# lRomul/ball-action-spotting

Hardware: AMD Instinct MI355X
Metric: frame-windows/sec (fwd+bwd) at 15x736x1280, batch 4 (higher is better)
Workload: dtype bf16; 1 GPU; sampling_weights_001: 4x15x736x1280 windows/GPU, fwd + focal loss + bwd + grad all-reduce + AdamW (mds.train fused focal loss / multi-tensor optimizer); global_batch=4, parallelism=dp1

## Files before the change

### ball-action-spotting_amd/csrc/k_pw.hip

```cpp
#include <stdlib.h>
#include "gemm.h"

#define PW_BM 128
#ifndef MDS_PW_GPRE3
#define MDS_PW_GPRE3 1
#endif
#define PW_BN 128
#define PW_SP 72

template <typename T> struct PwCfg;
template <> struct PwCfg<bf16_t> { static const int KC = 64, LD = 80; };
template <> struct PwCfg<float> { static const int KC = 32, LD = 40; };

template <typename T, int PRO, int WN, int BM, int TAIL, bool SPLIT = false, bool DEEP = false>
__global__ __launch_bounds__(256, (WN == 2 && BM == 128) || TAIL == 1 || SPLIT || DEEP ? 2 : 3) void pw_fwd_kernel(mds_pw_fwd_args a) {
  MDS_CHAIN_PRIO();
  static_assert(!DEEP || (TAIL != 1 && (PRO == MDS_PRO_NONE || PRO == MDS_PRO_GATE) && WN == 2 && BM == 64), "DEEP variants");
  static_assert(!SPLIT || (TAIL != 1 && (PRO == MDS_PRO_NONE || PRO == MDS_PRO_GATE) && WN == 2 && BM == 64), "SPLIT variants");
  constexpr bool POST = TAIL == 1, EPI = TAIL == 2;
  typedef typename Frag<T>::type frag_t;
  typedef Mma<T, EPI && sizeof(T) == 4 && MDS_EVAL_X3> MM;
  constexpr int KC = PwCfg<T>::KC, LD = PwCfg<T>::LD, VPR = KC / 8, RPP = 256 / VPR, NL = BM / RPP;
  constexpr int BN = 64 * WN, MFW = (WN == 2 ? BM / 32 : BM / 64), NLW = BN / RPP;
  MDS_DYN_SMEM(smem);
// ... 203 lines not shown
        const int last = t == (int)gridDim.z - 1;
        if (last) atomicExch(tk, 0);
        *lastp = last;
      }
      __syncthreads();
      const bool last = *lastp != 0;
      __syncthreads();
      if (!last) continue;
#pragma unroll
      for (int mf = 0; mf < MFW; ++mf)
#pragma unroll
        for (int nf = 0; nf < 4; ++nf) acc[mf][nf] = (f32x4){0.f, 0.f, 0.f, 0.f};
      for (int z0 = 0; z0 < (int)gridDim.z; z0 += 4) {
        f32x4 t[4][MFW][4];
#pragma unroll
        for (int zz = 0; zz < 4; ++zz)
#pragma unroll
          for (int mf = 0; mf < MFW; ++mf) {
            const long m = m0 + 16 * MFW * wm + 16 * mf + i;
            const bool ok = m < a.M && z0 + zz < (int)gridDim.z;
            const float* prow = a.split_part + (long)(z0 + zz) * MN + m * N + n0 + 64 * wn + 4 * q;
#pragma unroll
            for (int nf = 0; nf < 4; ++nf) t[zz][mf][nf] = (ok && nf < nfr) ? ld_coherent4(prow + 16 * nf) : (f32x4){0.f, 0.f, 0.f, 0.f};
          }
#pragma unroll
        for (int zz = 0; zz < 4; ++zz)
#pragma unroll
          for (int mf = 0; mf < MFW; ++mf)
#pragma unroll
            for (int nf = 0; nf < 4; ++nf) acc[mf][nf] += t[zz][mf][nf];
      }
    }

    float ps[16], pss[16];
#pragma unroll
    for (int e = 0; e < 16; ++e) { ps[e] = 0.f; pss[e] = 0.f; }
    float* pbn = (float*)smem;
    if (POST) {
      __syncthreads();
      if (tid < BN) {
#pragma unroll
        for (int k = 0; k < 4; ++k) pbn[k * BN + tid] = pb[k];
      }
      __syncthreads();
    }
    if (EPI) {
      __syncthreads();
      if (tid < BN) { pbn[tid] = pb[0]; pbn[BN + tid] = pb[1]; }
      __syncthreads();
    }
#pragma unroll
    for (int mf = 0; mf < MFW; ++mf) {
      const long m = m0 + 16 * MFW * wm + 16 * mf + i;
      const bool ok = m < a.M;
      T* yrow = y + (ok ? m : 0) * N + n0 + 64 * wn + 4 * q;
      float v[4][4];
#pragma unroll
      for (int nf = 0; nf < 4; ++nf)
#pragma unroll
        for (int r = 0; r < 4; ++r) v[nf][r] = acc[mf][nf][r];
      if (EPI) {
#pragma unroll
        for (int nf = 0; nf < 4; ++nf) {
          const float* pc = pbn + 64 * wn + 16 * nf + 4 * q;
          const f32x4 sc = *(const f32x4*)pc, sh = *(const f32x4*)(pc + BN);
#pragma unroll
          for (int r = 0; r < 4; ++r) {
            const float z = v[nf][r] * sc[r] + sh[r];
            v[nf][r] = a.epi.mode == MDS_EPI_BN_SILU ? siluf_(z) : z;
          }
        }
      }
      if (a.residual && ok) {
        const T* rrow = (const T*)a.residual + m * N + n0 + 64 * wn + 4 * q;
#pragma unroll
        for (int nf = 0; nf < 4; ++nf) {
          if (nf < nfr) {
            float rr[4];
            load4(rrow + 16 * nf, rr);
#pragma unroll
            for (int r = 0; r < 4; ++r) v[nf][r] += rr[r];
          }
        }
      }
      if (POST) {
        const float mk = (a.post.mode == MDS_POST_MASK) ? a.post.mask[(unsigned)(ok ? m : 0) / (unsigned)a.post.rows_per_group] : 1.0f;
#pragma unroll
        for (int nf = 0; nf < 4; ++nf) {
          if (nf < nfr) {
            const float ys[4] = {rys[mf][nf].get(0), rys[mf][nf].get(1), rys[mf][nf].get(2), rys[mf][nf].get(3)};
            const float* pc = pbn + 64 * wn + 16 * nf + 4 * q;
            const f32x4 mu = *(const f32x4*)(pc + 2 * BN), rs = *(const f32x4*)(pc + 3 * BN);
            if (a.post.mode == MDS_POST_SILU) {
              const f32x4 sc = *(const f32x4*)pc, sh = *(const f32x4*)(pc + BN);
#pragma unroll
              for (int r = 0; r < 4; ++r) v[nf][r] *= silu_gradf_(ys[r] * sc[r] + sh[r]);
            }
#pragma unroll
            for (int r = 0; r < 4; ++r) {
              const float g = Elem<T>::rnd(v[nf][r]) * mk;
              ps[nf * 4 + r] += g;
              pss[nf * 4 + r] += g * ((ys[r] - mu[r]) * rs[r]);
            }
          }
        }
      }
      if (STG) {
#pragma unroll
        for (int nf = 0; nf < 4; ++nf) store4(stg + i * PW_SP + 16 * nf + 4 * q, v[nf]);
        wave_lds_sync();
        T* ybase = y + (m0 + 16 * MFW * wm + 16 * mf) * N + n0 + 64 * wn;
#pragma unroll
        for (int t = 0; t < 2; ++t) {
          const int vv = lane + 64 * t, row = vv >> 3, c = vv & 7;
          if (m0 + 16 * MFW * wm + 16 * mf + row < a.M && (c >> 1) < nfr) {
            RawV8<T> o;
            o.ld(stg + row * PW_SP + 8 * c);
            o.st(ybase + (long)row * N + 8 * c);
          }
        }
        wave_lds_sync();
      } else if (ok) {
#pragma unroll
        for (int nf = 0; nf < 4; ++nf)
          if (nf < nfr) store4(yrow + 16 * nf, v[nf]);
      }
      if (!POST) {
#pragma unroll
        for (int nf = 0; nf < 4; ++nf)
#pragma unroll
          for (int r = 0; r < 4; ++r) { ps[nf * 4 + r] += v[nf][r]; pss[nf * 4 + r] += v[nf][r] * v[nf][r]; }
      }
    }
    if (POST ? (a.post.stats != nullptr) : (a.stats != nullptr)) {
      const int e = reduce_scatter16(ps, i);
      reduce_scatter16(pss, i);
      const int n = n0 + 64 * wn + 16 * (e >> 2) + 4 * q + (e & 3);
      if (n < N) {
        const long so = (long)((blockIdx.x + wm) % MDS_STAT_SLOTS) * 2 * N;
        if (POST) {
          atomicAdd(a.post.stats + so + n, (double)ps[0]);
          atomicAdd(a.post.stats + so + N + n, (double)pss[0]);
        } else {
          atomicAdd(a.stats + so + n, (double)ps[0]);
          atomicAdd(a.stats + so + N + n, (double)pss[0]);
        }
      }
    }
  }
}

int pw_fwd_wres_try(const mds_pw_fwd_args* a, mds_stream_t stream);
int pw_fwd_k_try(const mds_pw_fwd_args* a, mds_stream_t stream);

int c3_pw_try(const mds_pw_fwd_args* a, mds_stream_t stream);

extern "C" int mds_pw_fwd(const mds_pw_fwd_args* a, mds_stream_t stream) {
  MDS_REQUIRE(a && a->M > 0 && a->K > 0 && a->N > 0, "pw_fwd: bad dims");
  MDS_REQUIRE(a->K % 8 == 0 && a->N % 16 == 0, "pw_fwd: K=%d must be a multiple of 8, N=%d of 16", a->K, a->N);
  MDS_REQUIRE(a->x && a->w && a->y, "pw_fwd: null pointer");
  MDS_REQUIRE(a->pro.mode == MDS_PRO_NONE || a->pro.mode == MDS_PRO_GATE || (a->pro.scale && a->pro.shift), "pw_fwd: prologue needs scale/shift");
  MDS_REQUIRE((a->pro.mode != MDS_PRO_BN_SILU_GATE && a->pro.mode != MDS_PRO_GATE) || (a->pro.gate && a->pro.rows_per_group > 0), "pw_fwd: gate prologue");
  const bool post = a->post.mode != MDS_POST_NONE;
  const bool epi = a->epi.mode != MDS_EPI_NONE;
  if (epi) {
    MDS_REQUIRE(a->epi.scale && a->epi.shift && !a->stats && !post, "pw_fwd: an output transform needs scale/shift and excludes statistics and post statistics");
    MDS_REQUIRE(a->pro.mode == MDS_PRO_NONE || a->pro.mode == MDS_PRO_GATE || a->pro.mode == MDS_PRO_BN_SILU, "pw_fwd: an output transform takes the NONE, GATE or BN_SILU prologue");
  }
  if (post) {
    MDS_REQUIRE(a->post.y && a->post.bn && a->post.stats && !a->stats, "pw_fwd: post statistics need y, bn, stats (and no forward stats)");
    MDS_REQUIRE(a->post.mode != MDS_POST_MASK || (a->post.mask && a->post.rows_per_group > 0), "pw_fwd: post mask");
    MDS_REQUIRE(a->pro.mode == MDS_PRO_NONE && a->M < 4294967295L, "pw_fwd: post statistics are a data-gradient feature (no forward prologue)");
  }
  const bool split = a->split > 1;
  if (split) {
    MDS_REQUIRE(a->split <= MDS_PW_MAX_SPLIT && a->split_part && a->split_ticket, "pw_fwd: split-K needs split <= %d, a partial buffer and tickets", MDS_PW_MAX_SPLIT);
    MDS_REQUIRE(!post && !a->stats && (a->pro.mode == MDS_PRO_NONE || a->pro.mode == MDS_PRO_GATE),
                "pw_fwd: split-K is an inference-plan feature (NONE / GATE prologue, no statistics, no post statistics)");
  }
  if (!split && c3_pw_try(a, stream)) return mds_check_launch("pw_fwd");
  if (!split) { const int rc = pw_fwd_k_try(a, stream); if (rc <= 0) return rc; }
  if (!split) { const int rc = pw_fwd_wres_try(a, stream); if (rc <= 0) return rc; }
  const int wn = (a->N <= 64 && !split) ? 1 : 2;
  const int BN = 64 * wn;
  const long bar64 = mds_knob(MDS_KNOB_PW_BM64) > 0 ? 1000L * mds_knob(MDS_KNOB_PW_BM64) : 400000;
  const int bm = (wn == 2 && a->M <= bar64) ? 64 : PW_BM;
  MDS_REQUIRE(!split || bm == 64, "pw_fwd: split-K is for small M (64-row tiles)");
  const int mt = cdiv(a->M, bm), nt = cdiv(a->N, BN);
  int gy = 1;
  if (nt > 1) { gy = cdiv(mds_knob(MDS_KNOB_PW_GY) > 0 ? mds_knob(MDS_KNOB_PW_GY) : 1536, mt); if (gy > nt) gy = nt; if (gy < 1) gy = 1; }
  dim3 grid(mt, gy, split ? a->split : 1), block(256);
  const int kchunks = cdiv(split ? cdiv(a->K, a->split) : a->K, PwCfg<float>::KC);
  const bool deep = a->dtype == MDS_F32 && (epi || split) && wn == 2 && bm == 64 && kchunks >= 3 &&
                    (long)mt * gy * (split ? a->split : 1) <= 256 && mds_knob(MDS_KNOB_PW_DEEP) != 1;
#define PW_GOSPLIT(T, PRO, TAIL_) \
  do { const size_t smem = (size_t)(bm + BN) * PwCfg<T>::LD * sizeof(T) + (sizeof(T) == 2 ? 4 * 16 * PW_SP * 2 : 0); \
       if (sizeof(T) == 4 && deep) MDS_LAUNCH((pw_fwd_kernel<T, PRO, 2, 64, TAIL_, true, sizeof(T) == 4>), grid, block, smem, stream, *a); \
       else MDS_LAUNCH((pw_fwd_kernel<T, PRO, 2, 64, TAIL_, true>), grid, block, smem, stream, *a); } while (0)
#define PW_GODEEP(T, PRO) \
  do { const size_t smem = (size_t)(bm + BN) * PwCfg<T>::LD * sizeof(T) + (sizeof(T) == 2 ? 4 * 16 * PW_SP * 2 : 0); \
       MDS_LAUNCH((pw_fwd_kernel<T, PRO, 2, 64, 2, false, sizeof(T) == 4>), grid, block, smem, stream, *a); } while (0)
#define PW_GO2(T, PRO, TAIL_) \
  do { const size_t smem = (size_t)(bm + BN) * PwCfg<T>::LD * sizeof(T) + (sizeof(T) == 2 ? 4 * 16 * PW_SP * 2 : 0); \
       if (wn == 2 && bm == 64) MDS_LAUNCH((pw_fwd_kernel<T, PRO, 2, 64, TAIL_>), grid, block, smem, stream, *a); \
       else if (wn == 2) MDS_LAUNCH((pw_fwd_kernel<T, PRO, 2, 128, TAIL_>), grid, block, smem, stream, *a); \
       else MDS_LAUNCH((pw_fwd_kernel<T, PRO, 1, 128, TAIL_>), grid, block, smem, stream, *a); } while (0)
#define PW_GO(T, PRO) PW_GO2(T, PRO, 0)
  MDS_DISPATCH_DTYPE(a->dtype, T, {
    if (split) {
      if (epi) { if (a->pro.mode == MDS_PRO_GATE) PW_GOSPLIT(T, MDS_PRO_GATE, 2); else PW_GOSPLIT(T, MDS_PRO_NONE, 2); }
      else { if (a->pro.mode == MDS_PRO_GATE) PW_GOSPLIT(T, MDS_PRO_GATE, 0); else PW_GOSPLIT(T, MDS_PRO_NONE, 0); }
    }
    else if (post) PW_GO2(T, MDS_PRO_NONE, 1);
    else if (epi && deep && sizeof(T) == 4 && (a->pro.mode == MDS_PRO_GATE || a->pro.mode == MDS_PRO_NONE)) {
      if (a->pro.mode == MDS_PRO_GATE) PW_GODEEP(T, MDS_PRO_GATE); else PW_GODEEP(T, MDS_PRO_NONE);
    }
    else if (epi) { if (a->pro.mode == MDS_PRO_GATE) PW_GO2(T, MDS_PRO_GATE, 2); else if (a->pro.mode == MDS_PRO_BN_SILU) PW_GO2(T, MDS_PRO_BN_SILU, 2); else PW_GO2(T, MDS_PRO_NONE, 2); }
    else switch (a->pro.mode) {
      case MDS_PRO_NONE: PW_GO(T, MDS_PRO_NONE); break;
      case MDS_PRO_AFFINE: PW_GO(T, MDS_PRO_AFFINE); break;
      case MDS_PRO_BN_SILU: PW_GO(T, MDS_PRO_BN_SILU); break;
      case MDS_PRO_BN_SILU_GATE: PW_GO(T, MDS_PRO_BN_SILU_GATE); break;
      case MDS_PRO_GATE: PW_GO(T, MDS_PRO_GATE); break;
      default: mds_set_error("pw_fwd: prologue mode %d", a->pro.mode); return MDS_ERR_BAD_ARG;
    }
  });
#undef PW_GO
#undef PW_GO2
#undef PW_GOSPLIT
#undef PW_GODEEP
  return mds_check_launch("pw_fwd");
}

extern "C" int mds_pw_fwd_split(long M, int K, int N, int dtype) {
  const int knob = mds_knob(MDS_KNOB_PW_SPLIT);
  if (knob == 1 || M <= 0 || K <= 0 || N <= 0) return 1;
  const int kc = dtype == MDS_BF16 ? PwCfg<bf16_t>::KC : PwCfg<float>::KC;
  const long chunks = cdiv(K, kc), tiles = cdiv(M, MDS_PW_SPLIT_TILE_ROWS) * cdiv(N, 128);
  if (tiles >= 100 || chunks < 16) return 1;
  long s = knob >= 2 ? knob : 4;
  if (s > chunks / 3) s = chunks / 3;
  if (s > MDS_PW_MAX_SPLIT) s = MDS_PW_MAX_SPLIT;
  return s < 2 ? 1 : (int)s;
}

#define WG_ROWS 64
template <typename T> struct WgCfg;
template <> struct WgCfg<bf16_t> { static const int MW = 2, LDT = WG_ROWS + 8; };
template <> struct WgCfg<float> { static const int MW = 1, LDT = WG_ROWS + 4; };
template <int LDT> MDS_DEV int wg_off(int c, int m) { return c * LDT + 8 * ((m >> 3) ^ ((c >> 3) & 7)) + (m & 7); }
MDS_DEV void wg_put(bf16_t* base, int off, float v0, float v1) {
  *(uint32_t*)(base + off) = pack2(v0, v1);
}
MDS_DEV void wg_put(float* base, int off, float v0, float) { base[off] = v0; }

template <typename T, int PRO, int NF, int KF>
__global__ __launch_bounds__(256, 2) void pw_wgrad_kernel(mds_pw_wgrad_args a, int rows_per_block) {
  typedef typename Frag<T>::type frag_t;
  constexpr int MW = WgCfg<T>::MW, LDT = WgCfg<T>::LDT;
  constexpr int NT = 64 * NF, KT = 16 * KF, XCH = KT / 8, YCH = NT / 8;
  constexpr int XN = (WG_ROWS / MW) * XCH, YN = (WG_ROWS / MW) * YCH;
  constexpr int XI = (XN + 255) / 256, YI = (YN + 255) / 256;
  MDS_DYN_SMEM(smem);
  T* xsT = (T*)smem;
  T* dsT = xsT + KT * LDT;
  const int tid = threadIdx.x, lane = tid & 63, wave = MDS_UNIFORM(tid >> 6);
  const int i = lane & 15, q = lane >> 4;
  const int K = a.K, N = a.N;
  const int ntiles_k = (K + KT - 1) / KT;
  const int n0 = (blockIdx.y / ntiles_k) * NT, kt0 = (blockIdx.y % ntiles_k) * KT;
  const long mbeg = (long)blockIdx.x * rows_per_block;
  long mend = mbeg + rows_per_block;
  if (mend > a.M) mend = a.M;
  const T* x = (const T*)a.x;
  const T* dy = (const T*)a.dy;
  const int kfr = (K - kt0 >= KT) ? KF : ((K - kt0 + 15) >> 4);

  constexpr bool FIXED_CH = (256 % XCH) == 0;
  float sc[8], sh[8];
  if (FIXED_CH && PRO != MDS_PRO_NONE && PRO != MDS_PRO_GATE) {
    const int kx = kt0 + 8 * (tid % XCH);
    if (kx < K) { load8f(a.pro.scale + kx, sc); load8f(a.pro.shift + kx, sh); }
  }

  f32x4 acc[NF][KF];
#pragma unroll
  for (int u = 0; u < NF; ++u)
#pragma unroll
    for (int v = 0; v < KF; ++v) acc[u][v] = (f32x4){0.f, 0.f, 0.f, 0.f};

  RawV8<T> rx[XI][MW], ry[YI][MW];
  auto issue = [&](long mb) {
#pragma unroll
    for (int p = 0; p < XI; ++p) {
      const int it = tid + 256 * p, kx = kt0 + 8 * (it % XCH);
#pragma unroll
      for (int h = 0; h < MW; ++h) {
        const long m = mb + (it / XCH) * MW + h;
        if (it < XN && m < mend && kx < K) rx[p][h].ld(x + m * K + kx); else rx[p][h].zero();
      }
    }
#pragma unroll
    for (int p = 0; p < YI; ++p) {
      const int it = tid + 256 * p, n = n0 + 8 * (it % YCH);
#pragma unroll
      for (int h = 0; h < MW; ++h) {
        const long m = mb + (it / YCH) * MW + h;
        if (it < YN && m < mend && n < N) ry[p][h].ld(dy + m * N + n); else ry[p][h].zero();
      }
    }
  };
  issue(mbeg);
  for (long mb = mbeg; mb < mend; mb += WG_ROWS) {
    __syncthreads();
#pragma unroll
    for (int p = 0; p < XI; ++p) {
      const int it = tid + 256 * p, xc = it % XCH, kx = kt0 + 8 * xc;
      if (it < XN) {
        float v[MW][8];
#pragma unroll
        for (int h = 0; h < MW; ++h) {
          const long m = mb + (it / XCH) * MW + h;
          rx[p][h].get(v[h]);
          if (PRO != MDS_PRO_NONE && m < mend && kx < K) {
            if (PRO != MDS_PRO_GATE) {
              float scl[8], shl[8];
              if (!FIXED_CH) { load8f(a.pro.scale + kx, scl); load8f(a.pro.shift + kx, shl); }
#pragma unroll
              for (int j = 0; j < 8; ++j) {
                float z = v[h][j] * (FIXED_CH ? sc[j] : scl[j]) + (FIXED_CH ? sh[j] : shl[j]);
                v[h][j] = (PRO == MDS_PRO_AFFINE) ? z : siluf_(z);
              }
            }
            if (PRO == MDS_PRO_BN_SILU_GATE || PRO == MDS_PRO_GATE) {
// ... 268 lines not shown
```

### ball-action-spotting_amd/csrc/k_pwk8.hip

```cpp
#include <stdlib.h>
#include <type_traits>
#include "gemm.h"

namespace {
template <int V> using ic = std::integral_constant<int, V>;

template <int MFW, int WM, int NFW, int WN, int DX, int PRO, int TAIL>
__global__ __launch_bounds__(512) void pwk8_kernel(mds_pw_fwd_args a) {
  MDS_CHAIN_PRIO();
  static_assert(WM * WN == 4, "four consumer waves");
  constexpr bool XF = PRO != MDS_PRO_NONE;
  constexpr int NEED = XF ? 2 : 1;
  static_assert(DX >= NEED + 2, "at least one DMA batch stays in flight over a barrier");
  constexpr bool HAS_BN = PRO == MDS_PRO_AFFINE || PRO == MDS_PRO_BN_SILU || PRO == MDS_PRO_BN_SILU_GATE;
  constexpr bool HAS_ACT = PRO == MDS_PRO_BN_SILU || PRO == MDS_PRO_BN_SILU_GATE;
  constexpr bool HAS_GATE = PRO == MDS_PRO_BN_SILU_GATE || PRO == MDS_PRO_GATE;
  constexpr int BM = 16 * MFW * WM, BNP = 16 * NFW * WN;
  constexpr int NB = BM / 8;
  constexpr int XS = BM * 128, RX = DX + 1;
  constexpr int DW = 3;
  MDS_DYN_SMEM(smem);
  const lds_t xring = lds_addr_of(smem);
  const int tid = threadIdx.x, lane = tid & 63, wave = MDS_UNIFORM(tid >> 6);
  const long m0 = (long)blockIdx.x * BM;
// ... 204 lines not shown
    for (int nf = 0; nf < NFW; ++nf) {
      int f = wn * NFW + nf;
      if (f >= NFT) f = NFT - 1;
      wfp[nf] = (const bf16_t*)a.w_frag + (long)f * 512 + lane * 8;
    }
    const long wstep = (long)NFT * 512;
    u16x8 wf[4][NFW];
    int wk = 0;
    auto load_w = [&](auto Pc) {
      constexpr int P = decltype(Pc)::value;
      const int kk = wk < KST ? wk : KST - 1;
#pragma unroll
      for (int nf = 0; nf < NFW; ++nf) gld16(wf[P][nf], wfp[nf] + kk * wstep);
      ++wk;
    };
    const lds_t fo0 = wm * MFW * 2048 + i * 128 + ((q ^ (i & 7)) << 4), fo1 = wm * MFW * 2048 + i * 128 + (((4 + q) ^ (i & 7)) << 4);
    u16x8 xf[2][MFW];
    int csx = 0;

    load_w(ic<0>()); load_w(ic<1>()); load_w(ic<2>());
    for (int t = -NEED; t < 0; ++t) raw_barrier();
#pragma unroll
    for (int mf = 0; mf < MFW; ++mf) xf[0][mf] = lds_ld16(xring + mf * 2048 + fo0);

    auto kstep = [&](auto Pc, auto KSc, lds_t nxt, int s) {
      constexpr int P = decltype(Pc)::value, KS = decltype(KSc)::value;
      PWK_STAMP(s + NEED, 3 * KS);
      wait_vm<(DW - 1) * NFW>();
      wait_lgkm0();
      PWK_STAMP(s + NEED, 3 * KS + 1);
#pragma unroll
      for (int nf = 0; nf < NFW; ++nf) reg_pin(wf[P][nf]);
#pragma unroll
      for (int mf = 0; mf < MFW; ++mf) reg_pin(xf[KS][mf]);
      MDS_SCHED_FENCE();
      load_w(ic<(P + DW) & 3>());
      MDS_SCHED_FENCE();
#pragma unroll
      for (int nf = 0; nf < NFW; ++nf)
#pragma unroll
        for (int mf = 0; mf < MFW; ++mf) {
          mma16(wf[P][nf], xf[KS][mf], acc[mf][nf]);
          if (nf == 0) xf[KS ^ 1][mf] = lds_ld16(nxt + mf * 2048 + (KS ? fo0 : fo1));
          MDS_SCHED_FENCE();
        }
      PWK_STAMP(s + NEED, 3 * KS + 2);
    };
    auto stage = [&](int s, auto SPc) {
      constexpr int SP = decltype(SPc)::value;
      const lds_t xb = xring + csx * XS;
      int nsx = csx + 1;
      if (nsx == RX) nsx = 0;
      const lds_t xn = xring + nsx * XS;
      const bool last = s == S - 1, two = !(ktail && last);
      kstep(ic<2 * SP>(), ic<0>(), xb, s);
      raw_barrier();
      if (two) kstep(ic<2 * SP + 1>(), ic<1>(), xn, s);
      csx = nsx;
    };
    for (int s = 0; s < S; s += 2) {
      stage(s, ic<0>());
      if (s + 1 < S) stage(s + 1, ic<1>());
    }
    PWK_STAMP(S + NEED, 0);
    wait_vm<0>();
    wait_lgkm0();
  }
#ifdef PWK_TRACE
  raw_barrier();
  if (trc) {
    const unsigned long long* tl = (const unsigned long long*)(smem + RX * XS);
    for (int e = tid; e < (S + NEED + 1) * 64; e += 512) ((unsigned long long*)a.split_part)[e] = tl[e];
  }
  PWK_STAMP(S + NEED + 1, 0);
#endif

  raw_barrier();
  constexpr int SP = BNP + 4;
  float* stage_f = (float*)smem;
  if (wave < 4) {
    const int i = lane & 15, q = lane >> 4;
    const int wm = wave / WN, wn = wave % WN;
#pragma unroll
    for (int mf = 0; mf < MFW; ++mf)
#pragma unroll
      for (int nf = 0; nf < NFW; ++nf)
        *(f32x4*)(stage_f + (16 * (wm * MFW + mf) + i) * SP + 16 * (wn * NFW + nf) + 4 * q) = acc[mf][nf];
  }
  __syncthreads();
  if (rg < RG) {
#pragma unroll
    for (int jj = 0; jj < JMAX; ++jj) {
      const int rr = rg + RG * jj;
      const long m = m0 + rr;
      if (rr < BM && m < a.M) {
        const f32x4 lo4 = *(const f32x4*)(stage_f + rr * SP + 8 * c), hi4 = *(const f32x4*)(stage_f + rr * SP + 8 * c + 4);
        float v[8] = {lo4[0], lo4[1], lo4[2], lo4[3], hi4[0], hi4[1], hi4[2], hi4[3]};
        if (DG) {
#pragma unroll
          for (int j = 0; j < 8; ++j) {
            v[j] += bf2f(rres[jj][j]);
            if (post) {
              const float ys = bf2f(rys[jj][j]);
              if (a.post.mode == MDS_POST_SILU) v[j] *= silu_gradf_(ys * pb[0][j] + pb[1][j]);
              const float g = Elem<bf16_t>::rnd(v[j]) * rmk[jj];
              cs[j] += g;
              css[j] += g * ((ys - pb[2][j]) * pb[3][j]);
            }
          }
        } else {
#pragma unroll
          for (int j = 0; j < 8; ++j) { cs[j] += v[j]; css[j] += v[j] * v[j]; }
        }
        *(u16x8*)(y + m * N + 8 * c) = pack8(v);
      }
    }
  }
  if (sdst) {
    float* red = stage_f + BM * SP;
    if (rg < RG) {
      float* rp = red + (long)rg * 2 * N + 8 * c;
      *(f32x4*)rp = (f32x4){cs[0], cs[1], cs[2], cs[3]};
      *(f32x4*)(rp + 4) = (f32x4){cs[4], cs[5], cs[6], cs[7]};
      *(f32x4*)(rp + N) = (f32x4){css[0], css[1], css[2], css[3]};
      *(f32x4*)(rp + N + 4) = (f32x4){css[4], css[5], css[6], css[7]};
    }
    __syncthreads();
    double* sl = sdst + (long)(blockIdx.x % MDS_STAT_SLOTS) * 2 * N;
    for (int e = tid; e < 2 * N; e += 512) {
      float t = 0.f;
      for (int g = 0; g < RG; ++g) t += red[g * 2 * N + e];
      atomicAdd(sl + e, (double)t);
    }
  }
}

template <int MFW, int WM, int NFW, int WN, int DX>
size_t pwk8_smem(int N) {
  const int BM = 16 * MFW * WM, BNP = 16 * NFW * WN;
  size_t ring = (size_t)(DX + 1) * BM * 128;
#ifdef PWK_TRACE
  ring += 16 * 1024;
#endif
  const int RG = 512 / (N >> 3);
  const size_t epi = ((size_t)BM * (BNP + 4) + (size_t)RG * 2 * N) * 4;
  return ring > epi ? ring : epi;
}

bool pwk8_shape_ok(long M, int K, int N, int dtype) {
  return dtype == MDS_BF16 && K % 32 == 0 && K >= 64 && N % 16 == 0 && N <= 192 && N > 64 && M < 4294967295L;
}
}

extern "C" int mds_pw_fwd_wants_frag(long M, int K, int N, int dtype, int data_gradient) {
  const int knob = mds_knob(MDS_KNOB_PWK);
  if (knob == 1 || !pwk8_shape_ok(M, K, N, dtype)) return 0;
  if (knob == 2) return 1;
  if ((knob == 0 && data_gradient) || (knob == 4 && !data_gradient)) return 0;
  return K >= N && K >= 128 && N > 128 && M >= 4096 && M <= 40000;
}

int pw_fwd_k_try(const mds_pw_fwd_args* a, mds_stream_t stream) {
  if (!a->w_frag || a->epi.mode != MDS_EPI_NONE || a->split > 1) return 1;
  const int N = a->N, mode = a->pro.mode;
  const bool post = a->post.mode != MDS_POST_NONE;
  const bool dg = a->form ? a->form == 2 : (post || a->residual != nullptr);
  if (!dg && (post || a->residual != nullptr)) return 1;
  if (!mds_pw_fwd_wants_frag(a->M, a->K, a->N, a->dtype, dg)) return 1;
  if (dg && (mode != MDS_PRO_NONE || a->stats)) return 1;
  const int shape = N > 128 ? 0 : (N > 96 ? 1 : 2);
  const int cus = mds_cu_count();
  auto cost = [&](int bm) { const long blocks = cdiv(a->M, bm); return (long)cdiv(blocks, cus) * bm; };
  int BM;
  if (shape == 2) BM = 96;
  else { BM = 64; for (int bm : {80, 96, 128}) if (cost(bm) < cost(BM) && !(dg && bm > (shape == 0 ? 80 : 96))) BM = bm; }
  const int kb = mds_knob(MDS_KNOB_PWK_BM);
  if (kb > 0 && shape != 2 && (kb == 64 || kb == 80 || ((kb == 96 || kb == 128) && !(dg && kb > (shape == 0 ? 80 : 96))))) BM = kb;
  const bool gated = mode == MDS_PRO_BN_SILU_GATE || mode == MDS_PRO_GATE;
  if (gated && a->pro.rows_per_group < BM) return 1;
  const dim3 grid(cdiv(a->M, BM)), block(512);
#define PWK_GO(MFW, WM, NFW, WN, DX, PRO, TAIL)                                                                  \
  do { const size_t smem = pwk8_smem<MFW, WM, NFW, WN, DX>(N);                                                   \
       MDS_LAUNCH((pwk8_kernel<MFW, WM, NFW, WN, DX, PRO, TAIL>), grid, block, smem, stream, *a); } while (0)
#define PWK_ROWS(NFW, WN, DX, PRO, TAIL)                                                                         \
  do { if (BM == 64) PWK_GO(4, 1, NFW, WN, DX, PRO, TAIL); else if (BM == 80) PWK_GO(5, 1, NFW, WN, DX, PRO, TAIL); \
       else if (BM == 96) PWK_GO(6, 1, NFW, WN, DX, PRO, TAIL); else PWK_GO(8, 1, NFW, WN, DX, PRO, TAIL); } while (0)
#define PWK_SHAPE(DX, PRO, TAIL)                                                                                 \
  do { if (shape == 0) PWK_ROWS(3, 4, DX, PRO, TAIL); else if (shape == 1) PWK_ROWS(2, 4, DX, PRO, TAIL);        \
       else PWK_GO(3, 2, 3, 2, DX, PRO, TAIL); } while (0)
  if (dg) {
    if (shape == 2) PWK_GO(3, 2, 3, 2, 6, MDS_PRO_NONE, 1);
    else if (BM == 64) { if (shape == 0) PWK_GO(4, 1, 3, 4, 6, MDS_PRO_NONE, 1); else PWK_GO(4, 1, 2, 4, 6, MDS_PRO_NONE, 1); }
    else if (BM == 80) { if (shape == 0) PWK_GO(5, 1, 3, 4, 6, MDS_PRO_NONE, 1); else PWK_GO(5, 1, 2, 4, 6, MDS_PRO_NONE, 1); }
    else PWK_GO(6, 1, 2, 4, 6, MDS_PRO_NONE, 1);
  }
  else switch (mode) {
    case MDS_PRO_NONE: PWK_SHAPE(6, MDS_PRO_NONE, 0); break;
    case MDS_PRO_AFFINE: PWK_SHAPE(7, MDS_PRO_AFFINE, 0); break;
    case MDS_PRO_BN_SILU: PWK_SHAPE(7, MDS_PRO_BN_SILU, 0); break;
    case MDS_PRO_BN_SILU_GATE: PWK_SHAPE(7, MDS_PRO_BN_SILU_GATE, 0); break;
    default: PWK_SHAPE(7, MDS_PRO_GATE, 0); break;
  }
#undef PWK_SHAPE
#undef PWK_ROWS
#undef PWK_GO
  return mds_check_launch("pw_fwd (K-streaming)");
}
```

### include/mds.h

```cpp
#ifndef MDS_H
#define MDS_H
#ifdef __cplusplus
extern "C" {
#endif

#define MDS_VERSION 133
#define MDS_F32 0
#define MDS_BF16 1
#define MDS_STAT_SLOTS 32

#define MDS_ERR_BAD_ARG (-1)
#define MDS_ERR_UNSUPPORTED (-2)
#define MDS_ERR_LAUNCH (-3)

typedef void* mds_stream_t;

int mds_version(void);
const char* mds_last_error(void);
#define MDS_KNOB_CONV_BLOCKS 0
#define MDS_KNOB_DW_ORDER 1
#define MDS_KNOB_PW_WRES 2
#define MDS_KNOB_WG_DBG 4
#define MDS_KNOB_WG_BLOCKS 5
#define MDS_KNOB_DW3_L 7
#define MDS_KNOB_STREAM_BLOCKS 8
#define MDS_KNOB_DW2_L 9
#define MDS_KNOB_PW_SPLIT 10
#define MDS_KNOB_DW2_R 11
#define MDS_KNOB_PW_GY 12
#define MDS_KNOB_PW_BM64 13
#define MDS_KNOB_REDUCE_PASSES 14
#define MDS_KNOB_DW2_BLOCKS 15
#define MDS_KNOB_REDUCE_BLOCKS 16
#define MDS_KNOB_PW_DEEP 17
#define MDS_KNOB_PWK 18
#define MDS_KNOB_PWK_BM 19
#define MDS_KNOB_STEM_FWD 20
#define MDS_KNOB_DW3G 21
#define MDS_KNOB_C3 22
#define MDS_KNOB_C3_BWD_BLOCKS 24
#define MDS_KNOB_COUNT 25
int mds_dev_set(int knob, int value);
int mds_launch_event(void* event);

#define MDS_EPI_NONE 0
#define MDS_EPI_AFFINE 1
#define MDS_EPI_BN_SILU 2
typedef struct {
  int mode;
  const float* scale;
  const float* shift;
} mds_epi_t;

#define MDS_PRO_NONE 0
#define MDS_PRO_AFFINE 1
#define MDS_PRO_BN_SILU 2
#define MDS_PRO_BN_SILU_GATE 3
#define MDS_PRO_GATE 4
typedef struct {
  int mode;
  const float* scale;
  const float* shift;
  const float* gate;
  long rows_per_group;
} mds_pro_t;

#define MDS_G_PLAIN 0
#define MDS_G_SILU 1
#define MDS_G_SE_SILU 2
#define MDS_G_MASK 3
typedef struct {
  int mode;
  const void* u;
  const float* gate;
  const float* dpooled;
  const float* mask;
  long rows_per_group;
} mds_gsrc_t;

typedef struct {
  int mode;
  mds_gsrc_t g;
  const void* y;
  const float* bn;
  const float* lin;
} mds_dyp_t;

#define MDS_POST_NONE 0
#define MDS_POST_PLAIN 1
#define MDS_POST_MASK 2
#define MDS_POST_SILU 3
typedef struct {
  int mode;
  const void* y;
  const float* bn;
  const float* mask;
  long rows_per_group;
  double* stats;
} mds_poststat_t;

typedef struct {
  int dtype;
  long M;
  int K, N;
  const void* x;
  const void* w;
  void* y;
  mds_pro_t pro;
  const void* residual;
  double* stats;
  mds_poststat_t post;
  mds_epi_t epi;
  const void* w_frag;
  int split;
  float* split_part;
  int* split_ticket;
  int form;
} mds_pw_fwd_args;
int mds_pw_fwd(const mds_pw_fwd_args* a, mds_stream_t stream);
int mds_pw_fwd_split(long M, int K, int N, int dtype);
int mds_pw_fwd_wants_frag(long M, int K, int N, int dtype, int data_gradient);
#define MDS_PW_MAX_SPLIT 16
#define MDS_PW_SPLIT_TILE_ROWS 64
#define MDS_PW_SPLIT_TICKET_STRIDE 32

typedef struct {
  int dtype;
  long M;
  int K, N;
  const void* x;
  const void* dy;
  float* dw;
  mds_pro_t pro;
} mds_pw_wgrad_args;
int mds_pw_wgrad(const mds_pw_wgrad_args* a, mds_stream_t stream);

#define MDS_MAX_TAPS 9
typedef struct {
  int dtype;
  int N, IH, IW, Cin;
  int OH, OW, Cout;
  int A, B;
  int oy0, ox0, os;
  int is;
  int ntaps;
  int dy[MDS_MAX_TAPS], dx[MDS_MAX_TAPS], wi[MDS_MAX_TAPS];
  int wtaps;
  const void* x;
  const void* w;
  void* y;
  mds_pro_t pro;
  const void* residual;
  double* stats;
  int ngroups;
  int g_ntaps[4], g_oy0[4], g_ox0[4], g_A[4], g_B[4];
  mds_epi_t epi;
  mds_poststat_t post;
} mds_conv_fwd_args;
int mds_conv_fwd(const mds_conv_fwd_args* a, mds_stream_t stream);
int mds_conv_dgrad_post_ok(int dtype, int N, int IH, int IW, int Cin, int Cout, int stride, int has_residual);

typedef struct {
  int dtype;
  int N, IH, IW, Cin, OH, OW, Cout;
  int is, ntaps;
  int dy[MDS_MAX_TAPS], dx[MDS_MAX_TAPS], wi[MDS_MAX_TAPS];
  int wtaps;
  const void* x;
  const void* dyt;
  float* dw;
  mds_pro_t pro;
} mds_conv_wgrad_args;
int mds_conv_wgrad(const mds_conv_wgrad_args* a, mds_stream_t stream);

typedef struct {
  const unsigned char* u8;
  int nsrc, src_h, src_w;
  int pad_top, pad_left;
  float scale;
} mds_ingest_t;
typedef struct {
  int dtype;
  int N, H, W, OH, OW, Cout;
  int pad_t, pad_l;
  const float* x;
  const void* w;
  void* y;
  double* stats;
  mds_ingest_t ingest;
  mds_epi_t epi;
} mds_stem_fwd_args;
int mds_stem_fwd(const mds_stem_fwd_args* a, mds_stream_t stream);

typedef struct {
// ... 396 lines not shown
```

Before: 334.4 frame-windows/s.

## Add row-stationary pointwise GEMM kernel for small-K, wide-N expansion layers

Adds a new pointwise forward kernel that keeps a tile of input rows (K of 96 to 192) resident in registers and streams weight fragments through a register ring, looping over all output column tiles. Each output tile is staged through double-buffered LDS so global stores are coalesced, and per-channel BN statistics are accumulated in LDS and flushed once per block. This targets expansion convolutions with N of 384 or more, where reloading the input for each column tile is wasteful. The frag-weight request now also covers these shapes. The cost is extra dispatch logic and a new template set with MFW/KST variants.

```diff
diff --git a/ball-action-spotting_amd/csrc/k_pw.hip b/ball-action-spotting_amd/csrc/k_pw.hip
--- a/ball-action-spotting_amd/csrc/k_pw.hip
+++ b/ball-action-spotting_amd/csrc/k_pw.hip
@@ -379,6 +379,7 @@
 
 int pw_fwd_wres_try(const mds_pw_fwd_args* a, mds_stream_t stream);
 int pw_fwd_k_try(const mds_pw_fwd_args* a, mds_stream_t stream);
+int pw_fwd_x_try(const mds_pw_fwd_args* a, mds_stream_t stream);
 
 int c3_pw_try(const mds_pw_fwd_args* a, mds_stream_t stream);
 
@@ -407,6 +408,7 @@
   }
   if (!split && c3_pw_try(a, stream)) return mds_check_launch("pw_fwd");
   if (!split) { const int rc = pw_fwd_k_try(a, stream); if (rc <= 0) return rc; }
+  if (!split) { const int rc = pw_fwd_x_try(a, stream); if (rc <= 0) return rc; }
   if (!split) { const int rc = pw_fwd_wres_try(a, stream); if (rc <= 0) return rc; }
   const int wn = (a->N <= 64 && !split) ? 1 : 2;
   const int BN = 64 * wn;
diff --git a/ball-action-spotting_amd/csrc/k_pwk8.hip b/ball-action-spotting_amd/csrc/k_pwk8.hip
--- a/ball-action-spotting_amd/csrc/k_pwk8.hip
+++ b/ball-action-spotting_amd/csrc/k_pwk8.hip
@@ -380,12 +380,18 @@
 }
 }
 
-extern "C" int mds_pw_fwd_wants_frag(long M, int K, int N, int dtype, int data_gradient) {
+int pw_fwd_x_wants(long M, int K, int N, int dtype, int data_gradient);
+
+static int pwk8_wants(long M, int K, int N, int dtype, int data_gradient) {
   const int knob = mds_knob(MDS_KNOB_PWK);
   if (knob == 1 || !pwk8_shape_ok(M, K, N, dtype)) return 0;
   if (knob == 2) return 1;
   if ((knob == 0 && data_gradient) || (knob == 4 && !data_gradient)) return 0;
   return K >= N && K >= 128 && N > 128 && M >= 4096 && M <= 40000;
+}
+
+extern "C" int mds_pw_fwd_wants_frag(long M, int K, int N, int dtype, int data_gradient) {
+  return pwk8_wants(M, K, N, dtype, data_gradient) || pw_fwd_x_wants(M, K, N, dtype, data_gradient);
 }
 
 int pw_fwd_k_try(const mds_pw_fwd_args* a, mds_stream_t stream) {
@@ -394,7 +400,7 @@
   const bool post = a->post.mode != MDS_POST_NONE;
   const bool dg = a->form ? a->form == 2 : (post || a->residual != nullptr);
   if (!dg && (post || a->residual != nullptr)) return 1;
-  if (!mds_pw_fwd_wants_frag(a->M, a->K, a->N, a->dtype, dg)) return 1;
+  if (!pwk8_wants(a->M, a->K, a->N, a->dtype, dg)) return 1;
   if (dg && (mode != MDS_PRO_NONE || a->stats)) return 1;
   const int shape = N > 128 ? 0 : (N > 96 ? 1 : 2);
   const int cus = mds_cu_count();
diff --git a/ball-action-spotting_amd/csrc/k_pwx.hip b/ball-action-spotting_amd/csrc/k_pwx.hip
--- /dev/null
+++ b/ball-action-spotting_amd/csrc/k_pwx.hip
@@ -0,0 +1,199 @@
+#include <stdlib.h>
+#include <type_traits>
+#include "gemm.h"
+
+namespace {
+template <int MFW, int KST>
+struct PwxCfg {
+  static constexpr int BM = 16 * MFW, S = (KST + 1) / 2;
+  static constexpr int R = 2 * KST, DW = R - 1;
+  static constexpr int SPT = (BM * 16 + 511) / 512;
+  static constexpr int XB = S * BM * 128;
+  static constexpr int SP = 272;
+  static constexpr int STG = BM * SP;
+};
+
+template <int MFW, int KST>
+__global__ __launch_bounds__(512) void pwx_kernel(mds_pw_fwd_args a) {
+  MDS_CHAIN_PRIO();
+  typedef PwxCfg<MFW, KST> C;
+  constexpr int BM = C::BM, S = C::S, R = C::R, DW = C::DW, SPT = C::SPT;
+  MDS_DYN_SMEM(smem);
+  const lds_t xlds = lds_addr_of(smem);
+  char* const stg = smem + C::XB;
+  float* const red = (float*)(stg + 2 * C::STG);
+  const int tid = threadIdx.x, lane = tid & 63, wave = MDS_UNIFORM(tid >> 6);
+  const int i = lane & 15, q = lane >> 4;
+  const long m0 = (long)blockIdx.x * BM;
+  const int K = a.K, N = a.N, NFT = N >> 4, J = (NFT + 7) >> 3;
+  const int rows = (int)(a.M - m0 < BM ? a.M - m0 : BM);
+  const bf16_t* x = (const bf16_t*)a.x;
+  bf16_t* y = (bf16_t*)a.y;
+  double* const sdst = a.stats;
+
+  const bf16_t* wb = (const bf16_t*)a.w_frag + lane * 8;
+  u16x8 wf[R];
+  auto wload = [&](u16x8& dst, int j, int ks) {
+    int f = wave + 8 * j;
+    if (f > NFT - 1) f = NFT - 1;
+    gld16(dst, wb + ((long)ks * NFT + f) * 512);
+  };
+#pragma unroll
+  for (int g = 0; g < DW; ++g) wload(wf[g], g / KST, g % KST);
+
+  {
+    const int lr = lane >> 3, lo = (lane & 7) ^ lr;
+    constexpr int NB = BM / 8;
+    for (int b = wave; b < S * NB; b += 8) {
+      const int s = b / NB, rb = b - s * NB;
+      long row = m0 + 8 * rb + lr;
+      if (row >= a.M) row = a.M - 1;
+      int k = 64 * s + 8 * lo;
+      if (k > K - 8) k = K - 8;
+      glds16(x + row * K + k, xlds + s * BM * 128 + rb * 1024);
+    }
+  }
+  mds_wait_stores();
+  __syncthreads();
+#pragma unroll
+  for (int g = 0; g < DW; ++g) reg_pin(wf[g]);
+  u16x8 xf[MFW][KST];
+#pragma unroll
+  for (int mf = 0; mf < MFW; ++mf) {
+    const int r = 16 * mf + i;
+    const bool live = r < rows;
+#pragma unroll
+    for (int ks = 0; ks < KST; ++ks) {
+      const int o = 4 * (ks & 1) + q;
+      u16x8 v = *(const u16x8*)(smem + (ks >> 1) * BM * 128 + r * 128 + ((o ^ (r & 7)) << 4));
+      xf[mf][ks] = live ? v : (u16x8){0, 0, 0, 0, 0, 0, 0, 0};
+    }
+  }
+
+  auto do_round = [&](auto PARc, auto STEADYc, int j) {
+    constexpr int PAR = decltype(PARc)::value;
+    constexpr bool STEADY = decltype(STEADYc)::value;
+    f32x4 acc[MFW];
+#pragma unroll
+    for (int mf = 0; mf < MFW; ++mf) acc[mf] = (f32x4){0.f, 0.f, 0.f, 0.f};
+#pragma unroll
+    for (int ks = 0; ks < KST; ++ks) {
+      if (STEADY) {
+        if (ks < KST - 1) wait_vm<DW - 1 + 2 * SPT>();
+        else wait_vm<DW - 1 + SPT>();
+      } else {
+        wait_vm<DW - 1>();
+      }
+      const int set = PAR * KST + ks;
+      reg_pin(wf[set]);
+      MDS_SCHED_FENCE();
+      const int nset = (set + R - 1) % R;
+      if (ks == 0) wload(wf[nset], j + 1, KST - 1);
+      else wload(wf[nset], j + 2, ks - 1);
+      MDS_SCHED_FENCE();
+#pragma unroll
+      for (int mf = 0; mf < MFW; ++mf) mma16(wf[set], xf[mf][ks], acc[mf]);
+      MDS_SCHED_FENCE();
+    }
+    const int f = wave + 8 * j;
+    if (sdst && f < NFT) {
+      float cs[4], css[4];
+#pragma unroll
+      for (int r = 0; r < 4; ++r) {
+        float s = 0.f, ss = 0.f;
+#pragma unroll
+        for (int mf = 0; mf < MFW; ++mf) { s += acc[mf][r]; ss += acc[mf][r] * acc[mf][r]; }
+        cs[r] = sum_over_i16(s);
+        css[r] = sum_over_i16(ss);
+      }
+      if (i == 0) {
+#pragma unroll
+        for (int r = 0; r < 4; ++r) { red[16 * f + 4 * q + r] = cs[r]; red[N + 16 * f + 4 * q + r] = css[r]; }
+      }
+    }
+    char* const st = stg + PAR * C::STG;
+#pragma unroll
+    for (int mf = 0; mf < MFW; ++mf) {
+      const float v[4] = {acc[mf][0], acc[mf][1], acc[mf][2], acc[mf][3]};
+      store4((bf16_t*)(st + (16 * mf + i) * C::SP + (16 * wave + 4 * q) * 2), v);
+    }
+    wait_lgkm0();
+    raw_barrier();
+    asm volatile("" ::: "memory");
+    const int ncs = (N - 128 * j) >= 128 ? 16 : (N - 128 * j) >> 3;
+    const float rncs = 1.0f / ncs;
+    const int total = rows * ncs;
+    u16x8 ov[SPT];
+    int off[SPT];
+#pragma unroll
+    for (int u = 0; u < SPT; ++u) {
+      int sgi = tid + 512 * u;
+      if (sgi >= total) sgi -= total;
+      if (sgi > total - 1) sgi = total - 1;
+      const int r = fdiv(sgi, rncs), c = sgi - r * ncs;
+      ov[u] = *(const u16x8*)(st + r * C::SP + c * 16);
+      off[u] = r * N + 8 * c;
+    }
+    bf16_t* const yb = y + m0 * N + 128 * j;
+#pragma unroll
+    for (int u = 0; u < SPT; ++u) *(u16x8*)(yb + off[u]) = ov[u];
+  };
+
+  do_round(std::integral_constant<int, 0>(), std::false_type(), 0);
+  if (J > 1) do_round(std::integral_constant<int, 1>(), std::false_type(), 1);
+  for (int j = 2; j < J; j += 2) {
+    do_round(std::integral_constant<int, 0>(), std::true_type(), j);
+    if (j + 1 < J) do_round(std::integral_constant<int, 1>(), std::true_type(), j + 1);
+  }
+
+  if (sdst) {
+    __syncthreads();
+    double* sl = sdst + (long)(blockIdx.x % MDS_STAT_SLOTS) * 2 * N;
+    for (int e = tid; e < 2 * N; e += 512) atomicAdd(sl + e, (double)red[e]);
+  }
+}
+
+template <int MFW, int KST>
+size_t pwx_smem(int N) {
+  typedef PwxCfg<MFW, KST> C;
+  return (size_t)C::XB + 2 * (size_t)C::STG + 2 * (size_t)N * sizeof(float);
+}
+
+bool pwx_shape_ok(int K, int N, int dtype) {
+  return dtype == MDS_BF16 && K >= 96 && K <= 192 && K % 16 == 0 && N >= 384 && N % 16 == 0;
+}
+}
+
+int pw_fwd_x_wants(long M, int K, int N, int dtype, int data_gradient) {
+  const int knob = mds_knob(MDS_KNOB_PWX);
+  if (knob == 1 || !pwx_shape_ok(K, N, dtype) || M <= 0) return 0;
+  if (knob == 2 || knob == 64 || knob == 80 || knob == 96) return 1;
+  if (data_gradient && knob != 3) return 0;
+  return M >= 8000 && M <= 48000;
+}
+
+int pw_fwd_x_try(const mds_pw_fwd_args* a, mds_stream_t stream) {
+  if (!a->w_frag || a->pro.mode != MDS_PRO_NONE || a->epi.mode != MDS_EPI_NONE || a->residual || a->post.mode != MDS_POST_NONE ||
+      a->split > 1)
+    return 1;
+  const bool dg = a->form == 2;
+  if (dg && a->stats) return 1;
+  if (!pw_fwd_x_wants(a->M, a->K, a->N, a->dtype, dg)) return 1;
+  const int KST = (a->K + 31) / 32, knob = mds_knob(MDS_KNOB_PWX);
+  const int cus = mds_cu_count();
+  auto cost = [&](int bm) { const long blocks = cdiv(a->M, bm); return (long)cdiv(blocks, cus) * bm; };
+  int BM = 64;
+  for (int bm : {80, 96}) if (cost(bm) < cost(BM)) BM = bm;
+  if (knob == 64 || knob == 80 || knob == 96) BM = knob;
+  const dim3 grid(cdiv(a->M, BM)), block(512);
+#define PWX_GO(MFW, KST_) \
+  do { MDS_LAUNCH((pwx_kernel<MFW, KST_>), grid, block, (pwx_smem<MFW, KST_>(a->N)), stream, *a); } while (0)
+#define PWX_K(MFW) \
+  do { if (KST == 3) PWX_GO(MFW, 3); else if (KST == 4) PWX_GO(MFW, 4); else if (KST == 5) PWX_GO(MFW, 5); else PWX_GO(MFW, 6); } while (0)
+  if (BM == 64) PWX_K(4);
+  else if (BM == 80) PWX_K(5);
+  else PWX_K(6);
+#undef PWX_K
+#undef PWX_GO
+  return mds_check_launch("pw_fwd (row-stationary)");
+}
diff --git a/include/mds.h b/include/mds.h
--- a/include/mds.h
+++ b/include/mds.h
@@ -39,7 +39,8 @@
 #define MDS_KNOB_DW3G 21
 #define MDS_KNOB_C3 22
 #define MDS_KNOB_C3_BWD_BLOCKS 24
-#define MDS_KNOB_COUNT 25
+#define MDS_KNOB_PWX 25
+#define MDS_KNOB_COUNT 26
 int mds_dev_set(int knob, int value);
 int mds_launch_event(void* event);
 
```

Result: no change. 334.6 frame-windows/s (median of 3 runs) (+0.1%).
